# gpustack/gpustack

Measured on AMD Instinct MI355X. Metric: output tokens/sec (serving, continuous batching), higher is better.
Workload: dtype bfloat16; 1 GPU; model=llama-3-8b, global_batch=512, seq_len=384, parallelism=dp1, isl=256, osl=128, concurrency_per_gpu=512, warmup_steps_actual=164

## Files before the change

### gpustack_amd/models/llama.py

```python
from __future__ import annotations

from dataclasses import dataclass

import torch
import torch.nn.functional as F
from torch import nn

from .. import ops
from ..engine.config import EngineConfig, ModelSpec
from ..parallel import Communicator


@dataclass
class ForwardMeta:

    is_prefill: bool
    positions: torch.Tensor
    slot_mapping: torch.Tensor
    logits_indices: torch.Tensor
    seq_lens_list: list[int] | None = None
    tile_start: torch.Tensor | None = None
    tile_q0: torch.Tensor | None = None
    tile_len: torch.Tensor | None = None
    block_tables: torch.Tensor | None = None
    seq_lens: torch.Tensor | None = None
    num_prefill_tokens: int = 0
    suffix_meta: tuple | None = None
    lora: object | None = None
    cp: object | None = None
    fused_decode: bool = False


class W4Pack:

    __slots__ = ("qw", "sc", "zs", "shape")

    def __init__(self, qw, sc, zs):
        self.qw, self.sc, self.zs = qw, sc, zs
        self.shape = (qw.shape[0], qw.shape[1] * 2)


class Fp8Pack:

    __slots__ = ("qw", "ws", "shape")

    def __init__(self, qw, ws):
        self.qw, self.ws = qw, ws
        self.shape = tuple(qw.shape)


def qlinear(x, w, pack: "W4Pack | Fp8Pack | None", bias=None):
    if pack is None:
        return F.linear(x, w, bias)
    if isinstance(pack, Fp8Pack):
        return ops.fp8_linear(x, pack.qw, pack.ws, bias)
    if x.is_cuda:
        import os as _os

        hip = ops._load_hip()
        if (x.shape[0] <= 1024
                and _os.environ.get("GPUSTACK_AMD_W4_KERNEL", "0") == "1"):
            out = torch.empty(x.shape[0], pack.shape[0], dtype=x.dtype,
                              device=x.device)
            hip.w4_gemm(out, x.contiguous(), pack.qw, pack.sc, pack.zs)
            if bias is not None:
                out += bias
            return out
        wt = torch.empty(pack.shape, dtype=torch.bfloat16, device=x.device)
        hip.w4_dequant(wt, pack.qw, pack.sc, pack.zs)
        return F.linear(x, wt, bias)
    from .quantized import dequant_w4_runtime

    wt = dequant_w4_runtime(pack.qw, pack.sc, pack.zs).to(x.dtype)
    return F.linear(x, wt, bias)


class Attention(nn.Module):
    def __init__(self, spec: ModelSpec, tp_size: int, comm: Communicator,
                 dtype, layer_idx: int = 0):
        super().__init__()
        self.spec = spec
        self.comm = comm
        self.hq = spec.num_heads // tp_size
        self.hkv = max(1, spec.num_kv_heads // tp_size)
# ... 295 lines not shown
        o = F.linear(out.reshape(T, self.nh * self.dv), self.o_w)
        return self.comm.all_reduce(o)

    def _gpu_row_tables(self, meta: ForwardMeta, T: int, dev):
        if meta.is_prefill:
            reps, lens = [], []
            for i, L in enumerate(meta.seq_lens_list or []):
                reps.extend([i] * L)
                lens.extend(range(1, L + 1))
            bt = meta.block_tables[torch.tensor(reps, device=dev)]
            return bt, torch.tensor(lens, dtype=torch.int32, device=dev)
        if meta.suffix_meta is not None:
            _tiles, starts, hists, news = meta.suffix_meta
            reps, lens = [], []
            for i, (h, n) in enumerate(zip(hists, news)):
                reps.extend([i] * n)
                lens.extend(range(h + 1, h + n + 1))
            bt = meta.block_tables[torch.tensor(reps, device=dev)]
            return bt, torch.tensor(lens, dtype=torch.int32, device=dev)
        return meta.block_tables, meta.seq_lens

    def _segments(self, meta: ForwardMeta, lat_rows, k_cache):
        dev = lat_rows.device
        D = self.r + self.dr
        flat = k_cache.view(-1, D)
        bs = self.spec_block_size(k_cache)
        if meta.is_prefill:
            off = 0
            for L in (meta.seq_lens_list or []):
                rows = torch.arange(off, off + L, device=dev)
                yield rows, lat_rows[off:off + L], torch.arange(L, device=dev)
                off += L
            tp = meta.num_prefill_tokens or lat_rows.shape[0]
            if tp < lat_rows.shape[0]:
                for j in range(lat_rows.shape[0] - tp):
                    L = int(meta.seq_lens[j])
                    bt = meta.block_tables[j]
                    idx = (bt[torch.arange(L, device=dev) // bs].long() * bs
                           + torch.arange(L, device=dev) % bs)
                    yield (torch.tensor([tp + j], device=dev), flat[idx],
                           torch.tensor([L - 1], device=dev))
        elif meta.suffix_meta is not None:
            _tiles, starts, hists, news = meta.suffix_meta
            for i, (st, hist, n) in enumerate(zip(starts, hists, news)):
                L = hist + n
                bt = meta.block_tables[i]
                idx = (bt[torch.arange(L, device=dev) // bs].long() * bs
                       + torch.arange(L, device=dev) % bs)
                yield (torch.arange(st, st + n, device=dev), flat[idx],
                       torch.arange(hist, L, device=dev))
        else:
            for j in range(lat_rows.shape[0]):
                L = int(meta.seq_lens[j])
                bt = meta.block_tables[j]
                idx = (bt[torch.arange(L, device=dev) // bs].long() * bs
                       + torch.arange(L, device=dev) % bs)
                yield (torch.tensor([j], device=dev), flat[idx],
                       torch.tensor([L - 1], device=dev))

    @staticmethod
    def spec_block_size(k_cache):
        return k_cache.shape[2]


class MLP(nn.Module):

    def __init__(self, spec: ModelSpec, tp_size: int, comm: Communicator, dtype):
        super().__init__()
        self.comm = comm
        h = spec.hidden_size
        self.i = spec.intermediate_size // tp_size
        self.no_gate = spec.mlp_no_gate
        gu_rows = self.i if self.no_gate else 2 * self.i
        self.gate_up_w = nn.Parameter(torch.empty(gu_rows, h, dtype=dtype), requires_grad=False)
        self.down_w = nn.Parameter(torch.empty(h, self.i, dtype=dtype), requires_grad=False)
        self.gate_up_pack: W4Pack | None = None
        self.down_pack: W4Pack | None = None
        self.layer_idx = 0
        self._gu_projs = ([("up_proj", 0, self.i)] if self.no_gate else
                          [("gate_proj", 0, self.i), ("up_proj", self.i, self.i)])
        self._down_projs = [("down_proj", 0, h)]
        self.act = spec.mlp_act

    def forward(self, x, meta: ForwardMeta | None = None):
        gu = qlinear(x, self.gate_up_w, self.gate_up_pack)
        if meta is not None and meta.lora is not None:
            meta.lora.apply(self.layer_idx, x, gu, self._gu_projs)
        if self.no_gate:
            act = (torch.square(F.relu(gu)) if self.act == "relu2"
                   else F.silu(gu))
        elif self.act == "gelu_tanh":
            act = (F.gelu(gu[:, :self.i], approximate="tanh")
                   * gu[:, self.i:])
        else:
            act = torch.empty(x.shape[0], self.i, dtype=x.dtype,
                              device=x.device)
            ops.silu_and_mul(act, gu)
        down = (qlinear(act, self.down_w, self.down_pack)
                if self.down_pack is not None
                else ops.linear_auto(act, self.down_w))
        if meta is not None and meta.lora is not None:
            meta.lora.apply(self.layer_idx, act, down, self._down_projs)
        return self.comm.all_reduce(down)


class MoEMLP(nn.Module):

    def __init__(self, spec: ModelSpec, tp_size: int, comm: Communicator, dtype):
        super().__init__()
        self.comm = comm
        self.spec = spec
        h = spec.hidden_size
        self.e = spec.num_experts
        self.top_k = spec.num_experts_per_tok
        self.i = spec.moe_intermediate_size // tp_size
        self.router_w = nn.Parameter(torch.empty(self.e, h, dtype=dtype),
                                     requires_grad=False)
        self.gate_up_w = nn.Parameter(
            torch.empty(self.e, 2 * self.i, h, dtype=dtype), requires_grad=False)
        self.down_w = nn.Parameter(
            torch.empty(self.e, h, self.i, dtype=dtype), requires_grad=False)
        self.gate_up_packs: list | None = None
        self.down_packs: list | None = None
        if spec.router_mode == "sigmoid_bias" or spec.router_logit_bias:
            self.router_bias = nn.Parameter(
                torch.zeros(self.e, dtype=torch.float32), requires_grad=False)
        else:
            self.router_bias = None
        if spec.moe_bias:
            self.gate_up_b = nn.Parameter(
                torch.zeros(self.e, 2 * self.i, dtype=dtype),
                requires_grad=False)
            self.down_b = nn.Parameter(
                torch.zeros(self.e, h, dtype=dtype), requires_grad=False)
        else:
            self.gate_up_b = None
            self.down_b = None
        self.shared_gate_w = (
            nn.Parameter(torch.empty(1, h, dtype=dtype),
                         requires_grad=False)
            if spec.shared_expert_gated else None)
        if spec.n_shared_experts > 0:
            si = spec.moe_intermediate_size * spec.n_shared_experts // tp_size
            self.shared_i = si
            self.shared_gate_up_w = nn.Parameter(
                torch.empty(2 * si, h, dtype=dtype), requires_grad=False)
            self.shared_down_w = nn.Parameter(
                torch.empty(h, si, dtype=dtype), requires_grad=False)
        else:
            self.shared_gate_up_w = None

    def _routing_consts(self, T: int, device):
        cache = getattr(self, "_rc", None)
        if cache is None:
            cache = self._rc = {}
        c = cache.get(T)
        if c is None:
            flat_tok = torch.arange(T, device=device).repeat_interleave(self.top_k)
            ones = torch.ones(T * self.top_k, dtype=torch.int32, device=device)
            if T > 1024:
                return flat_tok, ones
            c = cache[T] = (flat_tok, ones)
        return c

    def forward(self, x, meta: ForwardMeta | None = None):
        T = x.shape[0]
        rw = getattr(self, "_router_w_f32", None)
        if rw is None or rw.device != x.device:
            self._router_w_f32 = self.router_w.float()
            rw = self._router_w_f32
        logits = F.linear(x.float(), rw)
        if self.spec.router_logit_bias and self.router_bias is not None:
            logits = logits + self.router_bias
        if self.spec.router_mode == "sigmoid_bias":
            scores = torch.sigmoid(logits)
            choice = scores + self.router_bias
            ng, tg = self.spec.n_group, self.spec.topk_group
            if ng > 1:
                gs = (choice.view(T, ng, self.e // ng)
                      .topk(2, dim=-1)[0].sum(dim=-1))
# ... 144 lines not shown
            dw, dp = self._expert_w("down", e)
            he = qlinear(act, dw, dp,
                         self.down_b[e] if (self.down_b is not None and tp0)
                         else None)
            contrib[rows] = he * flat_w[rows].unsqueeze(1)

    def _bmm_dispatch(self, x, contrib, flat_exp, flat_tok, flat_w,
                      cap: int | None = None):
        import os as _os

        dbg = _os.environ.get("GPUSTACK_AMD_MOE_DEBUG", "0") == "1"

        def _ck(tag):
            if dbg:
                torch.cuda.synchronize()
                print(f"bmm[{tag}] ok", flush=True)

        TK = flat_exp.numel()
        order = torch.argsort(flat_exp, stable=True)
        s_exp = flat_exp[order]
        s_tok = flat_tok[order]
        counts = torch.bincount(s_exp, minlength=self.e)
        if cap is None:
            cap = int(counts.max())
        if cap == 0:
            return
        cap = (cap + 63) // 64 * 64
        _ck(f"route cap={cap} TK={TK}")
        offs = counts.cumsum(0) - counts
        pos = torch.arange(TK, device=x.device) - offs[s_exp]
        xpad = x.new_zeros(self.e, cap, x.shape[1])
        xpad[s_exp, pos] = x[s_tok]
        _ck("xpad")
        gu = torch.bmm(xpad, self._bank("gate_up").transpose(1, 2))
        if self.gate_up_b is not None:
            gu = gu + self.gate_up_b.unsqueeze(1)
        _ck("bmm1")
        act = self._act_mul(gu.reshape(self.e * cap, 2 * self.i))
        _ck("silu")
        hd = torch.bmm(act.view(self.e, cap, self.i),
                       self._bank("down").transpose(1, 2))
        if self.down_b is not None and self.comm.tp_rank == 0:
            hd = hd + self.down_b.unsqueeze(1)
        _ck("bmm2")
        contrib[order] = hd[s_exp, pos] * flat_w[order].unsqueeze(1)
        _ck("combine")



def _layer_norm(out, x, w, eps):
    xf = x.float()
    mu = xf.mean(-1, keepdim=True)
    var = (xf - mu).pow(2).mean(-1, keepdim=True)
    out.copy_(((xf - mu) * torch.rsqrt(var + eps) * w.float()).to(x.dtype))


class DecoderLayer(nn.Module):
    def __init__(self, spec: ModelSpec, tp_size: int, comm: Communicator,
                 dtype, layer_idx: int = 0):
        super().__init__()
        self.spec = spec
        if spec.kv_lora_rank:
            self.attn = MLAAttention(spec, tp_size, comm, dtype,
                                     layer_idx=layer_idx)
        else:
            self.attn = Attention(spec, tp_size, comm, dtype,
                                  layer_idx=layer_idx)
        if spec.num_experts > 0 and layer_idx >= spec.first_k_dense_replace:
            self.mlp = MoEMLP(spec, tp_size, comm, dtype)
        else:
            self.mlp = MLP(spec, tp_size, comm, dtype)
        h = spec.hidden_size
        self.input_norm = nn.Parameter(torch.empty(h, dtype=dtype), requires_grad=False)
        self.post_attn_norm = nn.Parameter(torch.empty(h, dtype=dtype), requires_grad=False)
        if spec.sandwich_norms:
            self.pre_ff_norm = nn.Parameter(torch.empty(h, dtype=dtype),
                                            requires_grad=False)
            self.post_ff_norm = nn.Parameter(torch.empty(h, dtype=dtype),
                                             requires_grad=False)
        elif spec.norm_after:
            self.pre_ff_norm = self.post_ff_norm = None
        else:
            self.pre_ff_norm = self.post_ff_norm = None

    def forward(self, x, residual, meta, cos_sin, k_cache, v_cache):
        eps = self.spec.rms_norm_eps
        if self.spec.parallel_block:
            return self._forward_parallel(x, meta, cos_sin, k_cache,
                                          v_cache, eps)
        if self.spec.sandwich_norms:
            return self._forward_sandwich(x, meta, cos_sin, k_cache,
                                          v_cache, eps)
        if self.spec.norm_after:
            return self._forward_norm_after(x, meta, cos_sin, k_cache,
                                            v_cache, eps)
        if residual is None:
            residual = x
            h = torch.empty_like(x)
            ops.rms_norm(h, x, self.input_norm, eps)
        else:
            h = x
            ops.fused_add_rms_norm(h, residual, self.input_norm, eps)
        a = self.attn(h, meta, cos_sin, k_cache, v_cache)
        rm = self.spec.residual_multiplier
        if rm:
            a = a * rm
        ops.fused_add_rms_norm(a, residual, self.post_attn_norm, eps)
        m = self.mlp(a, meta)
        if rm:
            m = m * rm
        return m, residual

    def _forward_parallel(self, x, meta, cos_sin, k_cache, v_cache, eps):
        h = torch.empty_like(x)
        _layer_norm(h, x, self.input_norm, eps)
        a = self.attn(h, meta, cos_sin, k_cache, v_cache)
        m = self.mlp(h, meta)
        return x + a + m, None

    def _forward_norm_after(self, x, meta, cos_sin, k_cache, v_cache, eps):
        a = self.attn(x, meta, cos_sin, k_cache, v_cache)
        ops.rms_norm(a, a, self.input_norm, eps)
        x = x + a
        m = self.mlp(x, meta)
        ops.rms_norm(m, m, self.post_attn_norm, eps)
        return x + m, None

    def _forward_sandwich(self, x, meta, cos_sin, k_cache, v_cache, eps):
        h = torch.empty_like(x)
        ops.rms_norm(h, x, self.input_norm, eps)
        a = self.attn(h, meta, cos_sin, k_cache, v_cache)
        ops.rms_norm(a, a, self.post_attn_norm, eps)
        x = x + a
        ops.rms_norm(h, x, self.pre_ff_norm, eps)
        m = self.mlp(h, meta)
        ops.rms_norm(m, m, self.post_ff_norm, eps)
        return x + m, None


class LlamaForCausalLM(nn.Module):
    def __init__(self, cfg: EngineConfig, comm: Communicator, device):
        super().__init__()
        spec = cfg.spec
        self.spec = spec
        self.cfg = cfg
        self.comm = comm
        self.device = torch.device(device)
        dtype = getattr(torch, cfg.dtype)
        self.dtype = dtype
        pp, pr = comm.pp_size, comm.pp_rank
        part = getattr(cfg, "pp_partition", None)
        if part and len(part) == pp and sum(part) == spec.num_layers:
            counts = list(part)
        else:
            counts = [spec.num_layers // pp
                      + (1 if i < spec.num_layers % pp else 0)
                      for i in range(pp)]
        self.layer_offset = sum(counts[:pr])
        self.num_local_layers = counts[pr]
        first, last = comm.is_first_stage, comm.is_last_stage
        if first or (last and spec.tie_word_embeddings):
            self.embed = nn.Parameter(
                torch.empty(spec.vocab_size, spec.hidden_size, dtype=dtype),
                requires_grad=False)
        else:
            self.embed = None
        self.layers = nn.ModuleList(
            [DecoderLayer(spec, cfg.tp_size, comm, dtype,
                          layer_idx=self.layer_offset + i)
             for i in range(self.num_local_layers)]
        )
        for i, layer in enumerate(self.layers):
            layer.attn.layer_idx = self.layer_offset + i
            layer.mlp.layer_idx = self.layer_offset + i
        if last:
            self.final_norm = nn.Parameter(
                torch.empty(spec.hidden_size, dtype=dtype), requires_grad=False)
            if spec.tie_word_embeddings:
                self.lm_head = self.embed
            else:
                self.lm_head = nn.Parameter(
                    torch.empty(spec.vocab_size, spec.hidden_size, dtype=dtype),
                    requires_grad=False)
        else:
            self.final_norm = None
            self.lm_head = None
        self.lm_head_pack: W4Pack | None = None
        self.offload = None
        if spec.kv_lora_rank:
            cache = ops.build_cos_sin_cache(
                spec.qk_rope_head_dim, spec.qk_rope_head_dim,
                cfg.max_model_len,
                base=spec.rope_theta, scaling=spec.rope_scaling,
            )
        else:
            cache = ops.build_cos_sin_cache(
                spec.head_dim,
                int(spec.head_dim * spec.partial_rotary_factor),
                cfg.max_model_len,
                base=spec.rope_theta, scaling=spec.rope_scaling,
            )
        self.register_buffer("cos_sin", cache.to(device), persistent=False)
        if spec.rope_local_theta:
            local = ops.build_cos_sin_cache(
                spec.head_dim, spec.head_dim, cfg.max_model_len,
                base=spec.rope_local_theta,
            )
            self.register_buffer("cos_sin_local", local.to(device),
                                 persistent=False)
        else:
            self.cos_sin_local = None
        self.to(device)

    @torch.inference_mode()
    def forward(self, token_ids: torch.Tensor, meta: ForwardMeta, kv,
                return_hidden: bool = False, return_both: bool = False):
        if self.comm.pp_size > 1 and not self.comm.is_first_stage:
            x = self.comm.recv_hidden(
                (token_ids.shape[0], self.spec.hidden_size),
                self.dtype, self.device)
        else:
            x = F.embedding(token_ids, self.embed)
            if self.spec.embed_scale:
                x = x * torch.tensor(self.spec.embed_scale,
                                     dtype=x.dtype).item()
        residual = None
        off = self.offload
        if off is not None:
            off.begin()
        for i, layer in enumerate(self.layers):
            if off is not None and i >= off.first:
                off.bind(i)
            cs = (self.cos_sin_local
                  if (self.cos_sin_local is not None and layer.attn.window)
                  else self.cos_sin)
            x, residual = layer(x, residual, meta, cs, kv.k_caches[i], kv.v_caches[i])
        if self.comm.pp_size > 1 and not self.comm.is_last_stage:
            if residual is None:
                self.comm.send_hidden(x.contiguous())
            else:
                s = (x.float() + residual.float()).to(self.dtype)
                self.comm.send_hidden(s)
            return None
        if self.spec.norm_type == "layernorm":
            assert residual is None
            _layer_norm(x, x, self.final_norm, self.spec.rms_norm_eps)
        elif residual is None:
            ops.rms_norm(x, x, self.final_norm, self.spec.rms_norm_eps)
        else:
            ops.fused_add_rms_norm(x, residual, self.final_norm,
                                   self.spec.rms_norm_eps)
        if return_hidden:
            return x
        hidden = x[meta.logits_indices]
        logits = qlinear(hidden, self.lm_head, self.lm_head_pack)
        if self.spec.final_logit_softcap:
            cap = self.spec.final_logit_softcap
            logits = torch.tanh(logits / cap) * cap
        if self.spec.logits_scaling:
            logits = logits / self.spec.logits_scaling
        if self.spec.logits_multiplier:
            logits = logits * self.spec.logits_multiplier
        if return_both:
            return logits, hidden
        return logits
```

### gpustack_amd/ops/__init__.py

```python
from __future__ import annotations

import os

import torch

from . import torch_ref

_HIP = None
_HIP_ERR: str | None = None


def _load_hip():
    global _HIP, _HIP_ERR
    if _HIP is not None or _HIP_ERR is not None:
        return _HIP
    try:
        import importlib.util
        from pathlib import Path

        so = Path(__file__).resolve().parent / "_hip_ops.so"
        if not so.exists():
            raise ImportError(
                f"{so} not found — build it with `python -m gpustack_amd.ops.build` "
                "(hipcc --offload-arch=gfx950)"
# ... 201 lines not shown
        torch_ref.varlen_prefill_attn(out, q, k, v, seq_lens, scale,
                                      sinks=sinks, window=window,
                                      softcap=softcap)


def build_paged_prefill_tiles(seq_starts: list[int], seq_hists: list[int],
                              seq_news: list[int], device):
    qstart, q0s, hists, news, seqi = [], [], [], [], []
    for i, (st, h, n) in enumerate(zip(seq_starts, seq_hists, seq_news)):
        for q0 in range(0, n, _PREFILL_BQ):
            qstart.append(st)
            q0s.append(q0)
            hists.append(h)
            news.append(n)
            seqi.append(i)
    mk = lambda a: torch.tensor(a, dtype=torch.int32, device=device)
    return mk(qstart), mk(q0s), mk(hists), mk(news), mk(seqi)


def paged_prefill_attn(out, q, k_cache, v_cache, block_tables,
                       seq_starts: list[int], seq_hists: list[int],
                       seq_news: list[int], scale: float, tiles=None,
                       sinks=None, window: int = 0,
                       softcap: float = 0.0) -> None:
    hip = _backend(q)
    if hip is not None:
        _require_validated_variant("paged-prefill", q, sinks, window,
                                   softcap)
        if tiles is None:
            tiles = build_paged_prefill_tiles(seq_starts, seq_hists,
                                              seq_news, q.device)
        hip.flash_prefill_paged(out, q, k_cache, v_cache, block_tables,
                                tiles[0], tiles[1], tiles[2], tiles[3],
                                tiles[4], scale, sinks=_sinks_f32(sinks),
                                window=window, softcap=softcap)
    else:
        torch_ref.paged_prefill_attn(out, q, k_cache, v_cache, block_tables,
                                     seq_starts, seq_hists, seq_news, scale,
                                     sinks=sinks, window=window,
                                     softcap=softcap)


_SG_WORKSPACES: dict = {}
_SPLITK_SHARED_FLOATS = 256 * 256 * 128


def _splitk_workspace(need_floats: int, device):
    device = torch.device(device)
    size = _SPLITK_SHARED_FLOATS
    if need_floats > size:
        size = 1 << (need_floats - 1).bit_length()
    key = (size, device.type, device.index)
    ws = _SG_WORKSPACES.get(key)
    if ws is None:
        ws = torch.empty(size, dtype=torch.float32, device=device)
        _SG_WORKSPACES[key] = ws
    return ws


def gemm8(x, w, out=None, safe: bool = False):
    import torch.nn.functional as F

    M, K = x.shape
    N = w.shape[0]
    if not x.is_cuda or N % 256 != 0 or K % 128 != 0:
        return F.linear(x, w, None)
    if out is None:
        out = torch.empty(M, N, dtype=x.dtype, device=x.device)
    hip = _backend(x)
    if hip is None:
        return F.linear(x, w, None)
    hip.gemm8(out, x.contiguous(), w, 1 if safe else 0)
    return out


def skinny_gemm(x, w, out=None, splitk: int | None = None, version: int = 1):
    import torch.nn.functional as F

    M, K = x.shape
    N = w.shape[0]
    if not x.is_cuda or N % 128 != 0 or K % 64 != 0:
        return F.linear(x, w, None)
    if splitk is None:
        mt = (M + 255) // 256
        nt = N // 128
        splitk = 1
        while (mt * nt * splitk < 400 and splitk < 8
               and K % (64 * splitk * 2) == 0):
            splitk *= 2
    if out is None:
        out = torch.empty(M, N, dtype=x.dtype, device=x.device)
    ws = _splitk_workspace(splitk * M * N, x.device) if splitk > 1 else None
    _load_hip().skinny_gemm(out, x, w, ws, splitk, version)
    return out


def linear_auto(x, w):
    import os

    import torch.nn.functional as F

    if (x.is_cuda and x.dim() == 2
            and os.environ.get("GPUSTACK_AMD_SKINNY_GEMM", "1") == "1"):
        M, K = x.shape
        N = w.shape[0]
        if (N == 4096 and K >= 8192 and 384 <= M <= 1024
                and K % 256 == 0 and x.stride(1) == 1):
            return skinny_gemm(x, w, splitk=4)
    return F.linear(x, w)


def mfma_probe(a, b):
    return _load_hip().mfma_probe(a, b)



FP8_KERNEL_MAX_M = 16384


def quantize_fp8_weight(w):
    return torch_ref.quantize_fp8_weight(w)


def fp8_quant_rows(x, xq=None, xs=None):
    M, K = x.shape
    if xq is None:
        xq = torch.empty(M, K, dtype=torch.float8_e4m3fn, device=x.device)
    if xs is None:
        xs = torch.empty(M, dtype=torch.float32, device=x.device)
    hip = _backend(x)
    if hip is not None:
        hip.fp8_quant_rows(xq, xs, x)
    else:
        torch_ref.fp8_quant_rows(xq, xs, x)
    return xq, xs


def fp8_dequant(q, out=None):
    if out is None:
        out = torch.empty(q.shape, dtype=torch.bfloat16, device=q.device)
    hip = _backend(q)
    if hip is not None:
        hip.fp8_dequant(out, q)
    else:
        torch_ref.fp8_dequant(out, q)
    return out


def fp8_gemm_splitk(M: int, N: int, K: int) -> int:
    blocks = ((M + 63) // 64 if M <= 64 else (M + 255) // 256) * (N // 128)
    limit = 512 if M <= 64 else 256
    splitk = 1
    while (blocks * splitk * 2 <= limit and splitk < 8
           and K % (128 * splitk * 2) == 0):
        splitk *= 2
    return splitk


def fp8_gemm(xq, xs, wq, ws, out=None, splitk: int | None = None):
    M, K = xq.shape
    N = wq.shape[0]
    if out is None:
        out = torch.empty(M, N, dtype=torch.bfloat16, device=xq.device)
    hip = _backend(xq)
    if hip is None:
        torch_ref.fp8_gemm(out, xq, xs, wq, ws)
        return out
    if splitk is None:
        splitk = fp8_gemm_splitk(M, N, K)
    wsp = _splitk_workspace(splitk * M * N, xq.device) if splitk > 1 else None
    hip.fp8_gemm(out, xq, xs, wq, ws, wsp, splitk)
    return out


def fp8_linear(x, qw, ws, bias=None):
    hip = _backend(x)
    if hip is None:
        return torch_ref.fp8_linear(x, qw, ws, bias)
    import torch.nn.functional as F

    xb = x if x.dtype == torch.bfloat16 else x.to(torch.bfloat16)
    xq, xs = fp8_quant_rows(xb.contiguous())
    M = xq.shape[0]
    force = os.environ.get("GPUSTACK_AMD_FP8_KERNEL")
    if force == "1" or (force != "0" and M <= FP8_KERNEL_MAX_M):
        out = fp8_gemm(xq, xs, qw, ws)
    else:
        out = F.linear(fp8_dequant(xq), fp8_dequant(qw))
        hip.fp8_scale_out(out, xs, ws)
    if out.dtype != x.dtype:
        out = out.to(x.dtype)
    if bias is not None:
# ... 6 lines not shown
```

### gpustack_amd/ops/csrc/bindings.cpp

```cpp
#include <torch/extension.h>
#include <c10/hip/HIPStream.h>
#include <hip/hip_runtime.h>

void rms_norm_launch(void*, const void*, const void*, float, int, int, hipStream_t);
void fused_add_rms_norm_launch(void*, void*, const void*, float, int, int, hipStream_t);
void rope_neox_launch(const long*, void*, void*, const float*, int, int, int, int, int, long, long, hipStream_t);
void silu_and_mul_launch(void*, const void*, long, int, hipStream_t);
void reshape_and_cache_launch(const void*, const void*, void*, void*, const long*, int, int, int, int, long, long, int, hipStream_t);
void greedy_sample_launch(long*, const void*, int, int, hipStream_t);
void sample_launch(long*, const void*, const float*, const int*, const float*, const float*, const long*, const long*, int, int, hipStream_t);
void mla_decode_launch(float*, const void*, const void*, const int*, const int*, int, int, int, int, int, int, float, int*, hipStream_t);
void paged_attn_decode_launch(void*, const void*, const void*, const void*, const int*, const int*, int, int, int, int, int, float, long, int, const float*, int, float, int*, hipStream_t);
void paged_attn_decode_fused_launch(void*, const void*, const void*, const void*, void*, void*, const long*, const float*, const long*, const int*, const int*, int, int, int, int, int, float, long, long, long, int*, hipStream_t);
void flash_prefill_launch(void*, const void*, const void*, const void*, const int*, const int*, const int*, int, int, int, int, int, float, long, long, long, const float*, int, float, int*, hipStream_t);
void flash_prefill_paged_launch(void*, const void*, const void*, const void*, const int*, const int*, const int*, const int*, const int*, const int*, int, int, int, int, int, float, long, const float*, int, float, int*, hipStream_t);
void mfma_probe_launch(float*, const void*, const void*, hipStream_t);
void skinny_gemm_launch(void*, const void*, const void*, void*, int, int, int, int, hipStream_t);
void gemm8_launch(void*, const void*, const void*, int, int, int, int, int*, hipStream_t);
void skinny_gemm_v2_launch(void*, const void*, const void*, void*, int, int, int, int, hipStream_t);
void gemm_lab_launch(void*, const void*, const void*, int, int, int, int, int*, hipStream_t);
void moe_gate_up_silu_launch(void*, const void*, const void*, const int*, const int*, const int*, const void*, int, int, int, int, int*, hipStream_t);
void moe_down_scale_launch(void*, const void*, const void*, const int*, const int*, const int*, const float*, const void*, int, int, int, int*, hipStream_t);
void w4_gemm_launch(void*, const void*, const void*, const void*, const void*, int, int, int, int*, hipStream_t);
void w4_dequant_launch(void*, const void*, const void*, const void*, long, int, int*, hipStream_t);
void fp8_gemm_launch(void*, const void*, const void*, const void*, const void*, void*, int, int, int, int, int*, hipStream_t);
void fp8_quant_rows_launch(void*, void*, const void*, int, int, int*, hipStream_t);
void fp8_dequant_launch(void*, const void*, long, hipStream_t);
void fp8_scale_out_launch(void*, const void*, const void*, long, int, int*, hipStream_t);
void fp8_mfma_probe_launch(float*, const void*, const void*, hipStream_t);

#define HIP_CHECK_LAST()                                                     \
  do {                                                                       \
    hipError_t e_ = hipGetLastError();                                       \
    TORCH_CHECK(e_ == hipSuccess, "HIP kernel launch failed: ",              \
                hipGetErrorString(e_));                                      \
  } while (0)

namespace {

hipStream_t cur_stream(const at::Tensor& t) {
  return c10::hip::getCurrentHIPStream(t.device().index()).stream();
}

void check_bf16(const at::Tensor& t, const char* name) {
  TORCH_CHECK(t.is_cuda(), name, " must be on GPU");
  TORCH_CHECK(t.scalar_type() == at::kBFloat16, name, " must be bf16");
  TORCH_CHECK(t.is_contiguous(), name, " must be contiguous");
}

bool is_fp8_cache(const at::Tensor& t) {
  return t.scalar_type() == at::kFloat8_e4m3fn || t.scalar_type() == at::kByte;
}

void check_cache(const at::Tensor& t, const char* name) {
  TORCH_CHECK(t.is_cuda(), name, " must be on GPU");
  TORCH_CHECK(t.scalar_type() == at::kBFloat16 || is_fp8_cache(t),
              name, " must be bf16 or fp8-e4m3");
  TORCH_CHECK(t.is_contiguous(), name, " must be contiguous");
}

long row_stride_3d(const at::Tensor& t, const char* name) {
  TORCH_CHECK(t.is_cuda(), name, " must be on GPU");
  TORCH_CHECK(t.scalar_type() == at::kBFloat16, name, " must be bf16");
  TORCH_CHECK(t.dim() == 3, name, " must be [T, H, D]");
  TORCH_CHECK(t.stride(2) == 1 && t.stride(1) == t.size(2),
              name, " heads/dims must be contiguous");
  return t.stride(0);
}

void rms_norm(at::Tensor out, at::Tensor input, at::Tensor weight, double eps) {
  check_bf16(out, "out"); check_bf16(input, "input"); check_bf16(weight, "weight");
  const int H = input.size(-1);
  const long T = input.numel() / H;
  TORCH_CHECK(H % 8 == 0, "hidden size must be a multiple of 8");
  rms_norm_launch(out.data_ptr(), input.data_ptr(), weight.data_ptr(),
                  (float)eps, (int)T, H, cur_stream(input));
  HIP_CHECK_LAST();
}

void fused_add_rms_norm(at::Tensor x, at::Tensor residual, at::Tensor weight,
                        double eps) {
  check_bf16(x, "x"); check_bf16(residual, "residual"); check_bf16(weight, "weight");
  const int H = x.size(-1);
  const long T = x.numel() / H;
  TORCH_CHECK(H % 8 == 0, "hidden size must be a multiple of 8");
  fused_add_rms_norm_launch(x.data_ptr(), residual.data_ptr(),
                            weight.data_ptr(), (float)eps, (int)T, H,
                            cur_stream(x));
  HIP_CHECK_LAST();
}

void rotary_embedding(at::Tensor positions, at::Tensor q, at::Tensor k,
                      at::Tensor cos_sin, long head_dim, long rot_dim) {
  const long qs = row_stride_3d(q, "q");
  const long ks = row_stride_3d(k, "k");
  TORCH_CHECK(positions.scalar_type() == at::kLong && positions.is_contiguous());
  TORCH_CHECK(cos_sin.scalar_type() == at::kFloat && cos_sin.is_contiguous());
  const int T = positions.size(0);
  const int D = (int)head_dim, R = (int)rot_dim;
  const int Hq = q.size(1);
  const int Hk = k.size(1);
  TORCH_CHECK((R / 2) % 8 == 0, "rot_dim/2 must be a multiple of 8");
// ... 185 lines not shown
  const long ks = row_stride_3d(k, "k");
  const long vs = row_stride_3d(v, "v");
  TORCH_CHECK(tile_start.scalar_type() == at::kInt && tile_start.is_contiguous());
  const int ntiles = tile_start.size(0);
  const int Hq = q.size(1), D = q.size(2), Hkv = k.size(1);
  const int DV = out.size(2);
  TORCH_CHECK(v.size(2) == DV, "v/out value dims must match");
  int err = 0;
  flash_prefill_launch(out.data_ptr(), q.data_ptr(), k.data_ptr(), v.data_ptr(),
                       tile_start.data_ptr<int>(), tile_q0.data_ptr<int>(),
                       tile_len.data_ptr<int>(), ntiles, Hq, Hkv, D, DV,
                       (float)scale, qs, ks, vs, sink_ptr_checked(sinks, Hq),
                       (int)window, (float)softcap, &err, cur_stream(q));
  TORCH_CHECK(!err, "flash_prefill: unsupported config D=", D, " DV=", DV);
  HIP_CHECK_LAST();
}

void flash_prefill_paged(at::Tensor out, at::Tensor q, at::Tensor k_cache,
                         at::Tensor v_cache, at::Tensor block_tables,
                         at::Tensor tile_qstart, at::Tensor tile_q0,
                         at::Tensor tile_hist, at::Tensor tile_new,
                         at::Tensor tile_seq, double scale,
                         c10::optional<at::Tensor> sinks, long window,
                         double softcap) {
  check_bf16(out, "out");
  const long qs = row_stride_3d(q, "q");
  check_bf16(k_cache, "k_cache"); check_bf16(v_cache, "v_cache");
  for (auto* t : {&block_tables, &tile_qstart, &tile_q0, &tile_hist,
                  &tile_new, &tile_seq}) {
    TORCH_CHECK(t->scalar_type() == at::kInt && t->is_contiguous());
  }
  const int ntiles = tile_qstart.size(0);
  const int Hq = q.size(1), D = q.size(2);
  const int Hkv = k_cache.size(1);
  TORCH_CHECK(k_cache.size(2) == 16, "paged prefill assumes block_size 16");
  const int maxb = block_tables.size(1);
  int err = 0;
  flash_prefill_paged_launch(
      out.data_ptr(), q.data_ptr(), k_cache.data_ptr(), v_cache.data_ptr(),
      block_tables.data_ptr<int>(), tile_qstart.data_ptr<int>(),
      tile_q0.data_ptr<int>(), tile_hist.data_ptr<int>(),
      tile_new.data_ptr<int>(), tile_seq.data_ptr<int>(), ntiles, Hq, Hkv, D,
      maxb, (float)scale, qs, sink_ptr_checked(sinks, Hq), (int)window,
      (float)softcap, &err, cur_stream(q));
  TORCH_CHECK(!err, "flash_prefill_paged: unsupported config D=", D);
  HIP_CHECK_LAST();
}

void gemm8(at::Tensor out, at::Tensor x, at::Tensor w, long safe) {
  check_bf16(out, "out"); check_bf16(x, "x"); check_bf16(w, "w");
  const int M = x.size(0), K = x.size(1), N = w.size(0);
  TORCH_CHECK(w.size(1) == K && out.size(0) == M && out.size(1) == N);
  int err = 0;
  gemm8_launch(out.data_ptr(), x.data_ptr(), w.data_ptr(), M, N, K,
               (int)safe, &err, cur_stream(x));
  TORCH_CHECK(!err, "gemm8: unsupported shape M=", M, " N=", N, " K=", K,
              " (need N%256==0, K%128==0)");
  HIP_CHECK_LAST();
}

void skinny_gemm(at::Tensor out, at::Tensor x, at::Tensor w,
                 c10::optional<at::Tensor> workspace, long splitk,
                 long version) {
  check_bf16(out, "out"); check_bf16(x, "x"); check_bf16(w, "w");
  const int M = x.size(0), K = x.size(1), N = w.size(0);
  TORCH_CHECK(w.size(1) == K && out.size(0) == M && out.size(1) == N);
  TORCH_CHECK(N % 128 == 0, "N must be a multiple of 128");
  TORCH_CHECK(K % (64 * splitk) == 0, "K must be a multiple of 64*splitk");
  void* ws = nullptr;
  if (splitk > 1) {
    TORCH_CHECK(workspace.has_value(), "splitk>1 needs an f32 workspace");
    TORCH_CHECK(workspace->scalar_type() == at::kFloat &&
                workspace->numel() >= (long)splitk * M * N);
    ws = workspace->data_ptr();
  }
  if (version == 2) {
    TORCH_CHECK(N % 256 == 0, "v2 needs N % 256 == 0");
    skinny_gemm_v2_launch(out.data_ptr(), x.data_ptr(), w.data_ptr(), ws, M,
                          N, K, (int)splitk, cur_stream(x));
  } else {
    skinny_gemm_launch(out.data_ptr(), x.data_ptr(), w.data_ptr(), ws, M, N,
                       K, (int)splitk, cur_stream(x));
  }
  HIP_CHECK_LAST();
}

void moe_gate_up_silu(at::Tensor act, at::Tensor x, at::Tensor w,
                      at::Tensor s_tok, at::Tensor offs, at::Tensor counts,
                      c10::optional<at::Tensor> bias, long act_mode) {
  check_bf16(act, "act"); check_bf16(x, "x"); check_bf16(w, "w");
  for (auto* t : {&s_tok, &offs, &counts}) {
    TORCH_CHECK(t->scalar_type() == at::kInt && t->is_contiguous());
  }
  const int E = w.size(0), H = x.size(1);
  const long I2 = w.size(1);
  const int I = (int)(I2 / 2);
  TORCH_CHECK(w.size(2) == H && act.size(1) == I);
  TORCH_CHECK(act.size(0) == s_tok.size(0));
  const void* bias_ptr = nullptr;
  if (bias.has_value()) {
    check_bf16(*bias, "bias");
    TORCH_CHECK(bias->numel() == (long)E * 2 * I, "gate_up bias must be [E, 2I]");
    bias_ptr = bias->data_ptr();
  }
  int err = 0;
  moe_gate_up_silu_launch(act.data_ptr(), x.data_ptr(), w.data_ptr(),
                          s_tok.data_ptr<int>(), offs.data_ptr<int>(),
                          counts.data_ptr<int>(), bias_ptr, (int)act_mode,
                          E, H, I, &err, cur_stream(x));
  TORCH_CHECK(!err, "moe_gate_up_silu: unsupported dims H=", H, " I=", I);
  HIP_CHECK_LAST();
}

void moe_down_scale(at::Tensor contrib, at::Tensor act, at::Tensor w,
                    at::Tensor offs, at::Tensor counts, at::Tensor order,
                    at::Tensor flat_w, c10::optional<at::Tensor> bias) {
  check_bf16(contrib, "contrib"); check_bf16(act, "act"); check_bf16(w, "w");
  for (auto* t : {&offs, &counts, &order}) {
    TORCH_CHECK(t->scalar_type() == at::kInt && t->is_contiguous());
  }
  TORCH_CHECK(flat_w.scalar_type() == at::kFloat && flat_w.is_contiguous());
  const int E = w.size(0), H = w.size(1), I = w.size(2);
  TORCH_CHECK(act.size(1) == I && contrib.size(1) == H);
  TORCH_CHECK(contrib.size(0) == order.size(0));
  const void* bias_ptr = nullptr;
  if (bias.has_value()) {
    check_bf16(*bias, "bias");
    TORCH_CHECK(bias->numel() == (long)E * H, "down bias must be [E, H]");
    bias_ptr = bias->data_ptr();
  }
  int err = 0;
  moe_down_scale_launch(contrib.data_ptr(), act.data_ptr(), w.data_ptr(),
                        offs.data_ptr<int>(), counts.data_ptr<int>(),
                        order.data_ptr<int>(), flat_w.data_ptr<float>(),
                        bias_ptr, E, H, I, &err, cur_stream(act));
  TORCH_CHECK(!err, "moe_down_scale: unsupported dims H=", H, " I=", I);
  HIP_CHECK_LAST();
}

void w4_gemm(at::Tensor out, at::Tensor x, at::Tensor qw, at::Tensor sc,
             at::Tensor zs) {
  check_bf16(out, "out"); check_bf16(x, "x");
  check_bf16(sc, "sc"); check_bf16(zs, "zs");
  TORCH_CHECK(qw.scalar_type() == at::kByte && qw.is_contiguous());
  const int M = x.size(0), K = x.size(1), N = qw.size(0);
  TORCH_CHECK(qw.size(1) == K / 2 && out.size(0) == M && out.size(1) == N);
  TORCH_CHECK(sc.size(0) == N && sc.size(1) == K / 128);
  int err = 0;
  w4_gemm_launch(out.data_ptr(), x.data_ptr(), qw.data_ptr(), sc.data_ptr(),
                 zs.data_ptr(), M, N, K, &err, cur_stream(x));
  TORCH_CHECK(!err, "w4_gemm: unsupported shape M=", M, " N=", N, " K=", K,
              " (need N%64==0, K%128==0)");
  HIP_CHECK_LAST();
}

void w4_dequant(at::Tensor out, at::Tensor qw, at::Tensor sc, at::Tensor zs) {
  check_bf16(out, "out"); check_bf16(sc, "sc"); check_bf16(zs, "zs");
  TORCH_CHECK(qw.scalar_type() == at::kByte && qw.is_contiguous());
  const long N = qw.size(0);
  const int K = (int)(qw.size(1) * 2);
  TORCH_CHECK(out.size(0) == N && out.size(1) == K);
  int err = 0;
  w4_dequant_launch(out.data_ptr(), qw.data_ptr(), sc.data_ptr(),
                    zs.data_ptr(), N, K, &err, cur_stream(out));
  TORCH_CHECK(!err, "w4_dequant: K must be a multiple of 128");
  HIP_CHECK_LAST();
// ... 62 lines not shown
void fp8_scale_out(at::Tensor out, at::Tensor xs, at::Tensor ws) {
  check_bf16(out, "out"); check_f32(xs, "xs"); check_f32(ws, "ws");
  TORCH_CHECK(out.dim() == 2);
  const long M = out.size(0);
  const int N = out.size(1);
  TORCH_CHECK(xs.numel() == M && ws.numel() == N);
  int err = 0;
  fp8_scale_out_launch(out.data_ptr(), xs.data_ptr(), ws.data_ptr(), M, N,
                       &err, cur_stream(out));
  TORCH_CHECK(!err, "fp8_scale_out: unsupported shape M=", M, " N=", N,
              " (need N%8==0)");
  HIP_CHECK_LAST();
}

at::Tensor fp8_mfma_probe(at::Tensor a, at::Tensor b) {
  check_fp8(a, "a"); check_fp8(b, "b");
  TORCH_CHECK(a.numel() == 16 * 32 && b.numel() == 32 * 16);
  auto d = at::zeros({16, 16}, a.options().dtype(at::kFloat));
  fp8_mfma_probe_launch(d.data_ptr<float>(), a.data_ptr(), b.data_ptr(),
                        cur_stream(a));
  HIP_CHECK_LAST();
  return d;
}

void gemm_lab(at::Tensor out, at::Tensor x, at::Tensor w, long mode) {
  check_bf16(out, "out"); check_bf16(x, "x"); check_bf16(w, "w");
  const int M = x.size(0), K = x.size(1), N = w.size(0);
  TORCH_CHECK(w.size(1) == K && out.size(0) == M && out.size(1) == N);
  int err = 0;
  gemm_lab_launch(out.data_ptr(), x.data_ptr(), w.data_ptr(), M, N, K,
                  (int)mode, &err, cur_stream(x));
  TORCH_CHECK(!err, "gemm_lab: unsupported shape/mode M=", M, " N=", N,
              " K=", K, " mode=", mode);
  HIP_CHECK_LAST();
}

at::Tensor mfma_probe(at::Tensor a, at::Tensor b) {
  check_bf16(a, "a"); check_bf16(b, "b");
  auto d = at::zeros({16, 16}, a.options().dtype(at::kFloat));
  mfma_probe_launch(d.data_ptr<float>(), a.data_ptr(), b.data_ptr(),
                    cur_stream(a));
  HIP_CHECK_LAST();
  return d;
}

}

#undef HIP_CHECK_LAST
PYBIND11_MODULE(TORCH_EXTENSION_NAME, m) {
  m.def("rms_norm", &rms_norm, "RMSNorm (bf16)");
  m.def("fused_add_rms_norm", &fused_add_rms_norm, "residual+=x; x=norm(residual)*w");
  m.def("rotary_embedding", &rotary_embedding, "in-place neox RoPE on q,k");
  m.def("silu_and_mul", &silu_and_mul, "silu(x[:d])*x[d:]");
  m.def("reshape_and_cache", &reshape_and_cache, "scatter K/V into paged pool");
  m.def("greedy_sample", &greedy_sample, "argmax over vocab");
  m.def("sample", &sample, "per-row top-k/top-p/min-p sampling");
  m.def("mla_decode", &mla_decode,
        "MLA absorbed decode over the paged latent cache (DeepSeek)");
  m.def("paged_attn_decode", &paged_attn_decode, "paged GQA decode attention",
        py::arg("out"), py::arg("q"), py::arg("k_cache"), py::arg("v_cache"),
        py::arg("block_tables"), py::arg("seq_lens"), py::arg("scale"),
        py::arg("sinks") = py::none(), py::arg("window") = 0,
        py::arg("softcap") = 0.0);
  m.def("paged_attn_decode_fused", &paged_attn_decode_fused,
        "neox rope + KV-cache write + paged GQA decode attention, one launch",
        py::arg("out"), py::arg("q"), py::arg("k"), py::arg("v"),
        py::arg("k_cache"), py::arg("v_cache"), py::arg("positions"),
        py::arg("cos_sin"), py::arg("slot_mapping"), py::arg("block_tables"),
        py::arg("seq_lens"), py::arg("scale"));
  m.def("flash_prefill", &flash_prefill, "varlen causal MFMA prefill attention",
        py::arg("out"), py::arg("q"), py::arg("k"), py::arg("v"),
        py::arg("tile_start"), py::arg("tile_q0"), py::arg("tile_len"),
        py::arg("scale"), py::arg("sinks") = py::none(),
        py::arg("window") = 0, py::arg("softcap") = 0.0);
  m.def("flash_prefill_paged", &flash_prefill_paged,
        py::arg("out"), py::arg("q"), py::arg("k_cache"), py::arg("v_cache"),
        py::arg("block_tables"), py::arg("tile_qstart"), py::arg("tile_q0"),
        py::arg("tile_hist"), py::arg("tile_new"), py::arg("tile_seq"),
        py::arg("scale"), py::arg("sinks") = py::none(),
        py::arg("window") = 0, py::arg("softcap") = 0.0,
        "MFMA prefill attention with paged-KV history (suffix/chunk rows)");
  m.def("mfma_probe", &mfma_probe, "16x16x32 bf16 MFMA layout probe");
  m.def("skinny_gemm", &skinny_gemm, "split-K skinny GEMM (bf16, f32 accum)");
  m.def("gemm8", &gemm8, "8-phase pipelined 256x256 GEMM (bf16, f32 accum)");
  m.def("gemm_lab", &gemm_lab, "GEMM schedule lab variants (A/B vs hipBLASLt)");
  m.def("moe_gate_up_silu", &moe_gate_up_silu,
        py::arg("act"), py::arg("x"), py::arg("w"), py::arg("s_tok"),
        py::arg("offs"), py::arg("counts"), py::arg("bias") = py::none(),
        py::arg("act_mode") = 0,
        "grouped MoE gate/up GEMM + SiLU (sorted assignments, sync-free)");
  m.def("moe_down_scale", &moe_down_scale,
        py::arg("contrib"), py::arg("act"), py::arg("w"), py::arg("offs"),
        py::arg("counts"), py::arg("order"), py::arg("flat_w"),
        py::arg("bias") = py::none(),
        "grouped MoE down GEMM + routing-weight scale/scatter");
  m.def("w4_gemm", &w4_gemm,
        "W4A16 GEMM: packed-int4 weights dequantized in-register");
  m.def("w4_dequant", &w4_dequant,
        "packed-int4 -> bf16 weight expansion (prefill transient)");
  m.def("fp8_quant_rows", &fp8_quant_rows,
        "per-row dynamic e4m3 quantization (codes + f32 scale per row)");
  m.def("fp8_gemm", &fp8_gemm,
        "W8A8 e4m3 GEMM, f32 accumulate, per-row x per-column scales");
  m.def("fp8_dequant", &fp8_dequant, "exact e4m3 -> bf16 up-conversion");
  m.def("fp8_scale_out", &fp8_scale_out,
        "in-place out[m,n] *= xs[m]*ws[n] (W8A8 fallback epilogue)");
  m.def("fp8_mfma_probe", &fp8_mfma_probe,
        "16x16x32 fp8 MFMA layout probe");
}
```

### gpustack_amd/ops/csrc/skinny_gemm.hip

```cpp
#include "splitk_tile.h"

namespace {

using namespace splitk;

constexpr int BM = 256;
constexpr int BK = ROW_BYTES / Bf16::ES;

template <bool WRITE_PARTIAL>
__global__ __launch_bounds__(THREADS) void skinny_gemm_kernel(
    void* __restrict__ out,
    const void* __restrict__ x,
    const float* __restrict__ xs,
    const void* __restrict__ w,
    const float* __restrict__ ws, int M, int N, int K, int splitk) {
  tile_body<Bf16, BM / 32, WRITE_PARTIAL>(out, x, xs, w, ws, M, N, K, splitk);
}

}

namespace {

constexpr int V2_BM = 256;
constexpr int V2_BN = 256;
// ... 18 lines not shown

  auto stage_phase = [&](int buf, int kb, int q) {
    const long kbase = tl.k0 + (long)kb * BK;
    const int row0 = (q < 2 ? tl.n0 : tl.m0) + (q & 1) * 128;
    if (q < 2)
      stage_rows<128, Bf16::ES, false>(
          Wl[buf] + (row0 % V2_BN) * ROW_BYTES, w, row0, N, K, kbase, t);
    else
      stage_rows<128, Bf16::ES, true>(
          Xl[buf] + (row0 % V2_BM) * ROW_BYTES, x, row0, M, K, kbase, t);
  };

  f32x4 acc[16][2];
#pragma unroll
  for (int mi = 0; mi < 16; ++mi)
#pragma unroll
    for (int ni = 0; ni < 2; ++ni) acc[mi][ni] = f32x4{0.f, 0.f, 0.f, 0.f};

#pragma unroll
  for (int q = 0; q < 4; ++q) stage_phase(0, 0, q);
  asm volatile("s_waitcnt vmcnt(0)" ::: "memory");
  __syncthreads();

  int buf = 0;
  for (int kb = 0; kb < tl.nk; ++kb) {
    const bool more = kb + 1 < tl.nk;
#pragma unroll
    for (int q = 0; q < 4; ++q) {
      if (more) stage_phase(buf ^ 1, kb + 1, q);
      i64x2 bfrag[2][2];
#pragma unroll
      for (int ni = 0; ni < 2; ++ni)
#pragma unroll
        for (int kk = 0; kk < 2; ++kk)
          bfrag[ni][kk] = read_frag(Wl[buf], wid * 32 + ni * 16 + lc,
                                    kk * 64 + lg * 16);
#pragma unroll
      for (int mi = 0; mi < 4; ++mi) {
        const int arow = q * 64 + mi * 16 + lc;
#pragma unroll
        for (int kk = 0; kk < 2; ++kk) {
          const i64x2 a = read_frag(Xl[buf], arow, kk * 64 + lg * 16);
          __builtin_amdgcn_s_setprio(1);
#pragma unroll
          for (int ni = 0; ni < 2; ++ni)
            acc[q * 4 + mi][ni] =
                Bf16::mma(a, bfrag[ni][kk], acc[q * 4 + mi][ni]);
          __builtin_amdgcn_s_setprio(0);
        }
      }
      if (more) {
        if (q == 1) asm volatile("s_waitcnt vmcnt(4)" ::: "memory");
        else if (q == 3) asm volatile("s_waitcnt vmcnt(2)" ::: "memory");
      } else if (q == 3) {
        asm volatile("s_waitcnt vmcnt(0)" ::: "memory");
      }
      __syncthreads();
    }
    buf ^= 1;
  }

  store_frags<false, WRITE_PARTIAL, false>(out, acc, xs, ws, tl.m0,
                                           tl.n0 + wid * 32, tl.split, M, N,
                                           lane);
}

}

void skinny_gemm_v2_launch(void* out, const void* x, const void* w,
                           void* workspace, int M, int N, int K, int splitk,
                           hipStream_t s) {
  launch<V2_BM, V2_BN, false>(skinny_gemm_v2_kernel<true>,
                              skinny_gemm_v2_kernel<false>, out, x, nullptr,
                              w, nullptr, workspace, M, N, K, splitk, s);
}

void skinny_gemm_launch(void* out, const void* x, const void* w,
                        void* workspace, int M, int N, int K, int splitk,
                        hipStream_t s) {
  launch<BM, BN, false>(skinny_gemm_kernel<true>, skinny_gemm_kernel<false>,
                        out, x, nullptr, w, nullptr, workspace, M, N, K,
                        splitk, s);
}
```

Baseline: 26670 tokens/s.

## Fuse MLP down-proj split-K reduce with next layer's residual add and RMSNorm

For dense single-GPU Llama layers with a skinny down projection, the split-K reduction of the down GEMM is merged into a kernel that also adds the residual and applies the next layer's input RMSNorm (or the final norm). The next layer then skips its own norm. This removes a separate split-K reduce pass and a fused_add_rms_norm launch per layer, along with their memory round trips, at the cost of cross-layer coupling and a slightly different accumulation order.

Result: no change. 26870 tokens/s (median of 4 runs) (+0.8%).

```diff
diff --git a/gpustack_amd/models/llama.py b/gpustack_amd/models/llama.py
--- a/gpustack_amd/models/llama.py
+++ b/gpustack_amd/models/llama.py
@@ -1,5 +1,6 @@
 from __future__ import annotations
 
+import os
 from dataclasses import dataclass
 
 import torch
@@ -461,7 +462,7 @@
         self._down_projs = [("down_proj", 0, h)]
         self.act = spec.mlp_act
 
-    def forward(self, x, meta: ForwardMeta | None = None):
+    def forward(self, x, meta: ForwardMeta | None = None, tail=None):
         gu = qlinear(x, self.gate_up_w, self.gate_up_pack)
         if meta is not None and meta.lora is not None:
             meta.lora.apply(self.layer_idx, x, gu, self._gu_projs)
@@ -475,6 +476,13 @@
             act = torch.empty(x.shape[0], self.i, dtype=x.dtype,
                               device=x.device)
             ops.silu_and_mul(act, gu)
+        if tail is not None:
+            residual, norm_w, eps = tail
+            gated = ops.skinny_gate(act.shape[0], self.down_w.shape[0],
+                                    act.shape[1], act.is_cuda)
+            return ops.mlp_down_add_rms_norm(
+                act, self.down_w, residual, norm_w, eps,
+                splitk=4 if gated else None)
         down = (qlinear(act, self.down_w, self.down_pack)
                 if self.down_pack is not None
                 else ops.linear_auto(act, self.down_w))
@@ -785,8 +793,26 @@
             self.pre_ff_norm = self.post_ff_norm = None
         else:
             self.pre_ff_norm = self.post_ff_norm = None
-
-    def forward(self, x, residual, meta, cos_sin, k_cache, v_cache):
+        self.tail_norm: tuple | None = None
+
+    def fuses_mlp_tail(self, rows: int, meta, is_cuda: bool) -> bool:
+        mode = os.environ.get("GPUSTACK_AMD_FUSED_MLP_TAIL", "1")
+        spec = self.spec
+        mlp = self.mlp
+        if (mode == "0" or self.tail_norm is None
+                or spec.parallel_block or spec.sandwich_norms
+                or spec.norm_after or spec.norm_type != "rmsnorm"
+                or spec.residual_multiplier
+                or not isinstance(mlp, MLP) or mlp.down_pack is not None
+                or mlp.comm.tp_size > 1
+                or (meta is not None and meta.lora is not None)):
+            return False
+        if mode == "force":
+            return True
+        return ops.skinny_gate(rows, spec.hidden_size, mlp.i, is_cuda)
+
+    def forward(self, x, residual, meta, cos_sin, k_cache, v_cache,
+                normed: bool = False, fuse_tail: bool = False):
         eps = self.spec.rms_norm_eps
         if self.spec.parallel_block:
             return self._forward_parallel(x, meta, cos_sin, k_cache,
@@ -797,7 +823,9 @@
         if self.spec.norm_after:
             return self._forward_norm_after(x, meta, cos_sin, k_cache,
                                             v_cache, eps)
-        if residual is None:
+        if normed:
+            h = x
+        elif residual is None:
             residual = x
             h = torch.empty_like(x)
             ops.rms_norm(h, x, self.input_norm, eps)
@@ -809,6 +837,10 @@
         if rm:
             a = a * rm
         ops.fused_add_rms_norm(a, residual, self.post_attn_norm, eps)
+        if fuse_tail:
+            owner, name = self.tail_norm
+            return self.mlp(a, meta, tail=(residual, getattr(owner, name),
+                                           eps)), residual
         m = self.mlp(a, meta)
         if rm:
             m = m * rm
@@ -876,6 +908,11 @@
         for i, layer in enumerate(self.layers):
             layer.attn.layer_idx = self.layer_offset + i
             layer.mlp.layer_idx = self.layer_offset + i
+        for i, layer in enumerate(self.layers):
+            if i + 1 < len(self.layers):
+                layer.tail_norm = (self.layers[i + 1], "input_norm")
+            elif last:
+                layer.tail_norm = (self, "final_norm")
         if last:
             self.final_norm = nn.Parameter(
                 torch.empty(spec.hidden_size, dtype=dtype), requires_grad=False)
@@ -928,6 +965,7 @@
                 x = x * torch.tensor(self.spec.embed_scale,
                                      dtype=x.dtype).item()
         residual = None
+        normed = False
         off = self.offload
         if off is not None:
             off.begin()
@@ -937,7 +975,10 @@
             cs = (self.cos_sin_local
                   if (self.cos_sin_local is not None and layer.attn.window)
                   else self.cos_sin)
-            x, residual = layer(x, residual, meta, cs, kv.k_caches[i], kv.v_caches[i])
+            fuse = layer.fuses_mlp_tail(x.shape[0], meta, x.is_cuda)
+            x, residual = layer(x, residual, meta, cs, kv.k_caches[i],
+                                kv.v_caches[i], normed=normed, fuse_tail=fuse)
+            normed = fuse
         if self.comm.pp_size > 1 and not self.comm.is_last_stage:
             if residual is None:
                 self.comm.send_hidden(x.contiguous())
@@ -945,7 +986,9 @@
                 s = (x.float() + residual.float()).to(self.dtype)
                 self.comm.send_hidden(s)
             return None
-        if self.spec.norm_type == "layernorm":
+        if normed:
+            pass
+        elif self.spec.norm_type == "layernorm":
             assert residual is None
             _layer_norm(x, x, self.final_norm, self.spec.rms_norm_eps)
         elif residual is None:
diff --git a/gpustack_amd/ops/__init__.py b/gpustack_amd/ops/__init__.py
--- a/gpustack_amd/ops/__init__.py
+++ b/gpustack_amd/ops/__init__.py
@@ -307,12 +307,7 @@
     if not x.is_cuda or N % 128 != 0 or K % 64 != 0:
         return F.linear(x, w, None)
     if splitk is None:
-        mt = (M + 255) // 256
-        nt = N // 128
-        splitk = 1
-        while (mt * nt * splitk < 400 and splitk < 8
-               and K % (64 * splitk * 2) == 0):
-            splitk *= 2
+        splitk = _skinny_splitk(M, N, K)
     if out is None:
         out = torch.empty(M, N, dtype=x.dtype, device=x.device)
     ws = _splitk_workspace(splitk * M * N, x.device) if splitk > 1 else None
@@ -320,19 +315,51 @@
     return out
 
 
+def _skinny_splitk(M: int, N: int, K: int) -> int:
+    mt = (M + 255) // 256
+    nt = N // 128
+    splitk = 1
+    while (mt * nt * splitk < 400 and splitk < 8
+           and K % (64 * splitk * 2) == 0):
+        splitk *= 2
+    return splitk
+
+
+def skinny_gate(M: int, N: int, K: int, is_cuda: bool) -> bool:
+    return (is_cuda
+            and os.environ.get("GPUSTACK_AMD_SKINNY_GEMM", "1") == "1"
+            and N == 4096 and K >= 8192 and 384 <= M <= 1024
+            and K % 256 == 0)
+
+
 def linear_auto(x, w):
-    import os
-
     import torch.nn.functional as F
 
-    if (x.is_cuda and x.dim() == 2
-            and os.environ.get("GPUSTACK_AMD_SKINNY_GEMM", "1") == "1"):
-        M, K = x.shape
-        N = w.shape[0]
-        if (N == 4096 and K >= 8192 and 384 <= M <= 1024
-                and K % 256 == 0 and x.stride(1) == 1):
-            return skinny_gemm(x, w, splitk=4)
+    if (x.dim() == 2 and x.stride(1) == 1
+            and skinny_gate(x.shape[0], w.shape[0], x.shape[1], x.is_cuda)):
+        return skinny_gemm(x, w, splitk=4)
     return F.linear(x, w)
+
+
+def mlp_down_add_rms_norm(x, w, residual, norm_w, eps: float,
+                          splitk: int | None = None):
+    M, K = x.shape
+    N = w.shape[0]
+    fusable = (x.is_cuda and x.dtype == torch.bfloat16 and N % 128 == 0
+               and N <= 8192 and K % 64 == 0 and M > 0
+               and x.is_contiguous() and residual.is_contiguous())
+    if fusable:
+        if splitk is None:
+            splitk = _skinny_splitk(M, N, K)
+        if splitk in (2, 4, 8) and K % (64 * splitk) == 0:
+            h = torch.empty(M, N, dtype=x.dtype, device=x.device)
+            ws = _splitk_workspace(splitk * M * N, x.device)
+            _load_hip().skinny_gemm_add_rms_norm(h, residual, x, w, norm_w,
+                                                 eps, ws, splitk)
+            return h
+    h = skinny_gemm(x, w, splitk=splitk)
+    fused_add_rms_norm(h, residual, norm_w, eps)
+    return h
 
 
 def mfma_probe(a, b):
diff --git a/gpustack_amd/ops/csrc/bindings.cpp b/gpustack_amd/ops/csrc/bindings.cpp
--- a/gpustack_amd/ops/csrc/bindings.cpp
+++ b/gpustack_amd/ops/csrc/bindings.cpp
@@ -18,6 +18,7 @@
 void skinny_gemm_launch(void*, const void*, const void*, void*, int, int, int, int, hipStream_t);
 void gemm8_launch(void*, const void*, const void*, int, int, int, int, int*, hipStream_t);
 void skinny_gemm_v2_launch(void*, const void*, const void*, void*, int, int, int, int, hipStream_t);
+bool skinny_gemm_add_rms_norm_launch(void*, void*, const void*, const void*, const void*, float, void*, int, int, int, int, hipStream_t);
 void gemm_lab_launch(void*, const void*, const void*, int, int, int, int, int*, hipStream_t);
 void moe_gate_up_silu_launch(void*, const void*, const void*, const int*, const int*, const int*, const void*, int, int, int, int, int*, hipStream_t);
 void moe_down_scale_launch(void*, const void*, const void*, const int*, const int*, const int*, const float*, const void*, int, int, int, int*, hipStream_t);
@@ -369,6 +370,36 @@
     skinny_gemm_launch(out.data_ptr(), x.data_ptr(), w.data_ptr(), ws, M, N,
                        K, (int)splitk, cur_stream(x));
   }
+  HIP_CHECK_LAST();
+}
+
+void skinny_gemm_add_rms_norm(at::Tensor h, at::Tensor residual, at::Tensor x,
+                              at::Tensor w, at::Tensor norm_w, double eps,
+                              at::Tensor workspace, long splitk) {
+  check_bf16(h, "h"); check_bf16(residual, "residual"); check_bf16(x, "x");
+  check_bf16(w, "w"); check_bf16(norm_w, "norm_w");
+  TORCH_CHECK(x.dim() == 2 && w.dim() == 2 && h.dim() == 2 &&
+              residual.dim() == 2);
+  const int M = x.size(0), K = x.size(1), N = w.size(0);
+  TORCH_CHECK(w.size(1) == K && h.size(0) == M && h.size(1) == N &&
+              residual.size(0) == M && residual.size(1) == N &&
+              norm_w.numel() == N);
+  TORCH_CHECK(N % 128 == 0, "N must be a multiple of 128");
+  TORCH_CHECK(N <= 8192, "N must be at most 8192 (row held in registers)");
+  TORCH_CHECK(splitk == 2 || splitk == 4 || splitk == 8,
+              "splitk must be 2, 4 or 8");
+  TORCH_CHECK(K % (64 * splitk) == 0, "K must be a multiple of 64*splitk");
+  TORCH_CHECK(workspace.is_cuda() && workspace.is_contiguous() &&
+              workspace.scalar_type() == at::kFloat &&
+              workspace.numel() >= (long)splitk * M * N,
+              "needs an f32 workspace of splitk*M*N");
+  if (M == 0) return;
+  const bool ok = skinny_gemm_add_rms_norm_launch(
+      h.data_ptr(), residual.data_ptr(), x.data_ptr(), w.data_ptr(),
+      norm_w.data_ptr(), (float)eps, workspace.data_ptr(), M, N, K,
+      (int)splitk, cur_stream(x));
+  TORCH_CHECK(ok, "skinny_gemm_add_rms_norm: no kernel for N=", N,
+              " splitk=", splitk);
   HIP_CHECK_LAST();
 }
 
@@ -597,6 +628,8 @@
         "MFMA prefill attention with paged-KV history (suffix/chunk rows)");
   m.def("mfma_probe", &mfma_probe, "16x16x32 bf16 MFMA layout probe");
   m.def("skinny_gemm", &skinny_gemm, "split-K skinny GEMM (bf16, f32 accum)");
+  m.def("skinny_gemm_add_rms_norm", &skinny_gemm_add_rms_norm,
+        "residual += x@w^T (split-K); h = norm(residual)*norm_w");
   m.def("gemm8", &gemm8, "8-phase pipelined 256x256 GEMM (bf16, f32 accum)");
   m.def("gemm_lab", &gemm_lab, "GEMM schedule lab variants (A/B vs hipBLASLt)");
   m.def("moe_gate_up_silu", &moe_gate_up_silu,
diff --git a/gpustack_amd/ops/csrc/skinny_gemm.hip b/gpustack_amd/ops/csrc/skinny_gemm.hip
--- a/gpustack_amd/ops/csrc/skinny_gemm.hip
+++ b/gpustack_amd/ops/csrc/skinny_gemm.hip
@@ -124,3 +124,122 @@
                         out, x, nullptr, w, nullptr, workspace, M, N, K,
                         splitk, s);
 }
+
+namespace {
+
+constexpr int TAIL_THREADS = 256;
+constexpr int TAIL_MAX_VEC = 4;
+
+template <int S, int SLOTS>
+__global__ __launch_bounds__(TAIL_THREADS) void
+splitk_reduce_add_rms_norm_kernel(unsigned short* __restrict__ h,
+                                  unsigned short* __restrict__ residual,
+                                  const float* __restrict__ partial,
+                                  const unsigned short* __restrict__ w,
+                                  float eps, int M, int N) {
+  const int nvec = N / 8;
+  const long MN = (long)M * N;
+  for (int row = blockIdx.x; row < M; row += gridDim.x) {
+    const float* pp = partial + (long)row * N;
+    unsigned short* rp = residual + (long)row * N;
+    unsigned short* hp = h + (long)row * N;
+    float vals[SLOTS][8];
+    float ss = 0.f;
+#pragma unroll
+    for (int slot = 0; slot < SLOTS; ++slot) {
+      const int v = threadIdx.x + slot * TAIL_THREADS;
+      if (v < nvec) {
+        f32x4 p[S][2];
+#pragma unroll
+        for (int s = 0; s < S; ++s) {
+          const f32x4* src =
+              reinterpret_cast<const f32x4*>(pp + s * MN + v * 8);
+          p[s][0] = src[0];
+          p[s][1] = src[1];
+        }
+        const u16x8 ur = *reinterpret_cast<const u16x8*>(rp + v * 8);
+        float f[8];
+#pragma unroll
+        for (int i = 0; i < 8; ++i) {
+          float a = 0.f;
+#pragma unroll
+          for (int s = 0; s < S; ++s) a += p[s][i >> 2][i & 3];
+          f[i] = bf2f(f2bf(a)) + bf2f(ur[i]);
+          vals[slot][i] = f[i];
+        }
+        {
+#pragma clang fp contract(off)
+          ss = __builtin_fmaf(f[0], f[0], ss);
+#pragma unroll
+          for (int i = 1; i < 7; ++i) {
+            const float q = f[i] * f[i];
+            ss = ss + q;
+          }
+          ss = __builtin_fmaf(f[7], f[7], ss);
+        }
+        *reinterpret_cast<u16x8*>(rp + v * 8) = f32_to_bf8(f);
+      }
+    }
+    __shared__ float red[TAIL_THREADS / WAVE_SIZE];
+    ss = wave_reduce_sum(ss);
+    if ((threadIdx.x & (WAVE_SIZE - 1)) == 0) red[threadIdx.x / WAVE_SIZE] = ss;
+    __syncthreads();
+    float tot = 0.f;
+#pragma unroll
+    for (int i = 0; i < TAIL_THREADS / WAVE_SIZE; ++i) tot += red[i];
+    const float inv = rsqrtf(tot / N + eps);
+#pragma unroll
+    for (int slot = 0; slot < SLOTS; ++slot) {
+      const int v = threadIdx.x + slot * TAIL_THREADS;
+      if (v < nvec) {
+        const u16x8 wv = *reinterpret_cast<const u16x8*>(w + v * 8);
+        float o[8];
+#pragma unroll
+        for (int i = 0; i < 8; ++i) o[i] = vals[slot][i] * inv * bf2f(wv[i]);
+        *reinterpret_cast<u16x8*>(hp + v * 8) = f32_to_bf8(o);
+      }
+    }
+    __syncthreads();
+  }
+}
+
+using TailKernel = void (*)(unsigned short*, unsigned short*, const float*,
+                            const unsigned short*, float, int, int);
+
+template <int S>
+TailKernel tail_kernel_for_slots(int slots) {
+  switch (slots) {
+    case 1: return splitk_reduce_add_rms_norm_kernel<S, 1>;
+    case 2: return splitk_reduce_add_rms_norm_kernel<S, 2>;
+    case 3: return splitk_reduce_add_rms_norm_kernel<S, 3>;
+    default: return splitk_reduce_add_rms_norm_kernel<S, 4>;
+  }
+}
+
+}
+
+bool skinny_gemm_add_rms_norm_launch(void* h, void* residual, const void* x,
+                                     const void* w, const void* norm_w,
+                                     float eps, void* workspace, int M, int N,
+                                     int K, int splitk, hipStream_t s) {
+  const int slots = (N / 8 + TAIL_THREADS - 1) / TAIL_THREADS;
+  if (N % 8 != 0 || slots < 1 || slots > TAIL_MAX_VEC) return false;
+  TailKernel tail;
+  switch (splitk) {
+    case 2: tail = tail_kernel_for_slots<2>(slots); break;
+    case 4: tail = tail_kernel_for_slots<4>(slots); break;
+    case 8: tail = tail_kernel_for_slots<8>(slots); break;
+    default: return false;
+  }
+  const int mt = (M + BM - 1) / BM;
+  const int nt = N / BN;
+  hipLaunchKernelGGL(skinny_gemm_kernel<true>, dim3(mt * nt * splitk),
+                     dim3(THREADS), 0, s, workspace, x, nullptr, w, nullptr,
+                     M, N, K, splitk);
+  const int grid = M < 8192 ? M : 8192;
+  hipLaunchKernelGGL(tail, dim3(grid), dim3(TAIL_THREADS), 0, s,
+                     (unsigned short*)h, (unsigned short*)residual,
+                     (const float*)workspace, (const unsigned short*)norm_w,
+                     eps, M, N);
+  return true;
+}
```
